# MIT-SPARK/Hydra-GNN

Hardware: AMD Instinct MI355X
Metric: scene-graphs/sec (fwd+bwd) MP3D hetero batch (higher is better)
Workload: dtype f32

## Files before the change

hydra-gnn_amd/csrc/front.hip:

```cpp
#include "device_fns.h"
#ifdef HMP_KTIME
#define PS_KT(i)                                                                           \
  do {                                                                                     \
    if (threadIdx.x == 0 && part == 0 && dir == 0 && J.ei == front_kt_ei) front_kt_slot(i); \
  } while (0)
namespace hmp {
__device__ const void* front_kt_ei;
__device__ void front_kt_slot(int i);
}
#endif
#include "plan_small.h"

namespace hmp {

KT_DEFINE(front)
#ifdef HMP_KTIME
__device__ void front_kt_slot(int i) { kt_buf[i] = wall_clock64(); }
#endif

typedef float f32x16 __attribute__((ext_vector_type(16)));

constexpr int FT = 64;
constexpr int FBK = 128;
constexpr int FLD = FBK + 2;
constexpr int FSTAGES = 3;
constexpr int F_STAGE_FLOATS = 2 * 2 * FT * FLD;
constexpr int F_RED_FLOATS = 16 * 16 * 64;
constexpr int F_GEMM_FLOATS = F_STAGE_FLOATS > F_RED_FLOATS ? F_STAGE_FLOATS : F_RED_FLOATS;
constexpr int F_SEG_OFF = F_GEMM_FLOATS * 4;
constexpr int F_GEMM_BYTES = F_SEG_OFF + FR_MAX_SEG * (int)sizeof(FrontSeg);
constexpr int F_LDS_BYTES = PS_LDS_BYTES > F_GEMM_BYTES ? PS_LDS_BYTES : F_GEMM_BYTES;

template <int VEC>
__device__ __forceinline__ float4 fr_ld4(const float* p, bool second_ok) {
  if (VEC == 4) return *reinterpret_cast<const float4*>(p);
  const float2 a = *reinterpret_cast<const float2*>(p);
  const float2 b = *reinterpret_cast<const float2*>(p + (second_ok ? 2 : 0));
  return make_float4(a.x, a.y, b.x, b.y);
}

template <int VEC, int NSRC>
__device__ __forceinline__ void front_gemm_tile(const FrontProb& P, const FrontSeg* __restrict__ sseg, const float* __restrict__ params,
                                                int tm, int tn, float* lds) {
  const int tid = threadIdx.x, lane = tid & 63, w = __builtin_amdgcn_readfirstlane(tid >> 6);
  const int m0 = tm * FT, n0 = tn * FT;
  const int k4 = (tid & 31) * 4;
  const float* arow[2];
  const float* brow[2][NSRC];
  int bn[2];
#pragma unroll
  for (int i = 0; i < 2; ++i) {
    const int row = (tid >> 5) + 32 * i;
    arow[i] = P.A + (int64_t)min(m0 + row, P.M - 1) * P.lda;
    const int c = n0 + row;
    int si = 0;
    while (si + 1 < P.n_seg && c >= sseg[si + 1].col0) ++si;
    const FrontSeg& S = sseg[si];
    const int br = c - S.col0;
    const bool blive = c < P.N && br >= 0 && br < S.rows;
    bn[i] = blive ? S.nsrc : 0;
#pragma unroll
    for (int q = 0; q < NSRC; ++q) brow[i][q] = params + S.off[q < S.nsrc ? q : 0] + (int64_t)(blive ? br : 0) * S.ld;
  }
  const int n_stage = (P.K + FBK - 1) / FBK;
  float4 ra[FSTAGES][2], rb[FSTAGES][2];
#pragma unroll
  for (int s = 0; s < FSTAGES; ++s) {
    const int gk = s * FBK + k4;
    const bool klive = s < n_stage && gk < P.K;
    const int kc = klive ? gk : 0;
    const bool sec = kc + 2 < P.K;
    const bool m1 = klive && gk + 1 < P.K, m2 = klive && gk + 2 < P.K, m3 = klive && gk + 3 < P.K;
#pragma unroll
    for (int i = 0; i < 2; ++i) {
      const float4 a = fr_ld4<VEC>(arow[i] + kc, sec);
      float4 b = fr_ld4<VEC>(brow[i][0] + kc, sec);
#pragma unroll
      for (int q = 1; q < NSRC; ++q) {
        const float4 t = fr_ld4<VEC>(brow[i][q] + kc, sec);
        if (q < bn[i]) { b.x += t.x; b.y += t.y; b.z += t.z; b.w += t.w; }
      }
      const bool bl = bn[i] > 0;
      ra[s][i] = make_float4(klive ? a.x : 0.f, m1 ? a.y : 0.f, m2 ? a.z : 0.f, m3 ? a.w : 0.f);
      rb[s][i] = make_float4(klive && bl ? b.x : 0.f, m1 && bl ? b.y : 0.f, m2 && bl ? b.z : 0.f, m3 && bl ? b.w : 0.f);
    }
  }
  KT(2);
  KTW(3);
  const int kg = w >> 2, sub = w & 3, wm = sub & 1, wn = sub >> 1;
  f32x16 acc;
#pragma unroll
  for (int i = 0; i < 16; ++i) acc[i] = 0.f;
  auto put = [&](int s) {
    float* As = lds + (s & 1) * (2 * FT * FLD);
    float* Bs = As + FT * FLD;
#pragma unroll
    for (int i = 0; i < 2; ++i) {
      const int row = (tid >> 5) + 32 * i;
      float2* pa = reinterpret_cast<float2*>(As + row * FLD + k4);
      float2* pb = reinterpret_cast<float2*>(Bs + row * FLD + k4);
      pa[0] = make_float2(ra[s][i].x, ra[s][i].y); pa[1] = make_float2(ra[s][i].z, ra[s][i].w);
      pb[0] = make_float2(rb[s][i].x, rb[s][i].y); pb[1] = make_float2(rb[s][i].z, rb[s][i].w);
    }
  };
  put(0);
  KT(5);
  __syncthreads();
  KT(6);
#pragma unroll
  for (int s = 0; s < FSTAGES; ++s) {
    if (s >= n_stage) break;
    if (s + 1 < FSTAGES && s + 1 < n_stage) put(s + 1);
    const float* As = lds + (s & 1) * (2 * FT * FLD);
    const float* Bs = As + FT * FLD;
    const int klen = min(FBK, P.K - s * FBK);
    const int nk = min(max(klen - kg * 32, 0), 32);
    const float* ap = As + (wm * 32 + (lane & 31)) * FLD + kg * 32 + (lane >> 5);
    const float* bp = Bs + (wn * 32 + (lane & 31)) * FLD + kg * 32 + (lane >> 5);
    if (nk == 32) {
#pragma unroll
      for (int h = 0; h < 2; ++h) {
        float av[8], bv[8];
#pragma unroll
        for (int i = 0; i < 8; ++i) {
          av[i] = ap[16 * h + 2 * i];
          bv[i] = bp[16 * h + 2 * i];
        }
#pragma unroll
        for (int i = 0; i < 8; ++i) acc = __builtin_amdgcn_mfma_f32_32x32x2f32(av[i], bv[i], acc, 0, 0, 0);
      }
    } else {
      for (int kk = 0; kk < nk; kk += 2) acc = __builtin_amdgcn_mfma_f32_32x32x2f32(ap[kk], bp[kk], acc, 0, 0, 0);
    }
    if (s == 0) KT(7);
    if (s == 1) KT(14);
    __syncthreads();
    if (s == 0) KT(13);
    if (s == 1) KT(15);
  }
  KT(4);
  float* red = lds;
#pragma unroll
  for (int i = 0; i < 16; ++i) red[(w * 16 + i) * 64 + lane] = acc[i];
  __syncthreads();
  const int col = n0 + wn * 32 + (lane & 31);
#pragma unroll
  for (int j = 0; j < 4; ++j) {
    const int i = 4 * kg + j;
    const float v = (red[((0 * 4 + sub) * 16 + i) * 64 + lane] + red[((1 * 4 + sub) * 16 + i) * 64 + lane]) +
                    (red[((2 * 4 + sub) * 16 + i) * 64 + lane] + red[((3 * 4 + sub) * 16 + i) * 64 + lane]);
    const int row = m0 + wm * 32 + j + 8 * kg + 4 * (lane >> 5);
    if (row < P.M && col < P.N) P.C[(int64_t)row * P.ldc + col] = v;
  }
}

template <int VEC>
__device__ __forceinline__ void front_gemm_v(const FrontProb& P, const FrontSeg* sseg, const float* params, int tm, int tn, float* lds) {
  switch (P.max_nsrc) {
    case 1: front_gemm_tile<VEC, 1>(P, sseg, params, tm, tn, lds); break;
    case 2: front_gemm_tile<VEC, 2>(P, sseg, params, tm, tn, lds); break;
    case 3: front_gemm_tile<VEC, 3>(P, sseg, params, tm, tn, lds); break;
    default: front_gemm_tile<VEC, FR_MAX_SRC>(P, sseg, params, tm, tn, lds); break;
  }
}

__global__ __launch_bounds__(1024) void front_kernel(const FrontArgs a) {
  __shared__ __attribute__((aligned(16))) char lds[F_LDS_BYTES];
  const int blk = blockIdx.x;
  if (blk < a.gemm_blocks) {
    KT(0);
    int pi = 0;
    while (pi + 1 < a.n_prob && blk >= a.prob_start[pi + 1]) ++pi;
    karg_warm<(sizeof(FrontProb) + 63) / 64 + 1>((int)offsetof(FrontArgs, prob) + pi * (int)sizeof(FrontProb), (int)sizeof(FrontProb));
    const FrontProb& P = a.prob[pi];
    const int local = blk - P.blk_start;
    const int tm = local / P.tiles_n, tn = local % P.tiles_n;
    FrontSeg* sseg = reinterpret_cast<FrontSeg*>(lds + F_SEG_OFF);
    if ((int)threadIdx.x < P.n_seg) sseg[threadIdx.x] = P.seg[threadIdx.x];
    __syncthreads();
    if (P.vec == 4) front_gemm_v<4>(P, sseg, a.params, tm, tn, reinterpret_cast<float*>(lds));
    else front_gemm_v<2>(P, sseg, a.params, tm, tn, reinterpret_cast<float*>(lds));
    KT(1);
    return;
  }
  if (blk < a.gemm_blocks + a.plan_blocks) {
    const int pb = blk - a.gemm_blocks;
    int jd = 0;
    while (jd + 1 < 2 * a.n_jobs && pb >= a.part_start[jd + 1]) ++jd;
    const FrontJob& F = a.job[jd >> 1];
    int* wsi = reinterpret_cast<int*>(a.ws);
    PlanJob J;
    J.ei = F.ei; J.E = F.E; J.n_src = F.n_src; J.n_dst = F.n_dst;
    J.rowptr = wsi + F.rowptr; J.col = wsi + F.col; J.eid = wsi + F.eid;
    J.t_rowptr = wsi + F.t_rowptr; J.t_col = wsi + F.t_col; J.t_pos = nullptr;
    J.degf = reinterpret_cast<float*>(wsi + F.degf);
    J.gp_dst = F.gp_dst; J.gp_src = F.gp_src; J.gp_edge = F.gp_edge; J.n_graphs = F.n_graphs;
    J.cnt_in = J.cnt_out = J.cur_in = J.cur_out = nullptr;
    J.tmpc_in = J.tmpc_out = nullptr;
    J.tmp_in = wsi + F.tmp_in; J.tmp_out = wsi + F.tmp_out; J.t_eid = wsi + F.t_eid; J.pos_of_eid = wsi + F.pos_of_eid;
#ifdef HMP_KTIME
    if (threadIdx.x == 0 && pb == 0) front_kt_ei = a.job[0].ei;
#endif
    const bool last = pb + 1 == a.part_start[jd + 1];
    if (a.plan_rc) plan_small_part<true>(J, jd & 1, pb - a.part_start[jd], a.rows_per_part[jd], last, a.need_tpos, a.status, lds);
    else plan_small_part<false>(J, jd & 1, pb - a.part_start[jd], a.rows_per_part[jd], last, a.need_tpos, a.status, lds);
    return;
  }
  const int kb = blk - a.gemm_blocks - a.plan_blocks;
  if (a.step_ctr && kb == 0 && threadIdx.x == 0) {
    const int t = *a.step_ctr + 1;
    *a.step_ctr = t;
    if (a.step_mirror) *a.step_mirror = t;
  }
  const int2 m = a.pack_map[kb];
  pack_item(a.segs[m.x], m.y + (int)(threadIdx.x >> 6), a.params, a.packed);
}

int front_launch(FrontArgs& a, hipStream_t st) {
  int start = 0;
  for (int i = 0; i < a.n_prob; ++i) {
    FrontProb& P = a.prob[i];
    HMP_CHECK_ARG(P.K >= 4 && P.K <= FSTAGES * FBK && (P.K & 1) == 0 && P.M > 0 && P.N > 0, "front: projection K %d unsupported", P.K);
    HMP_CHECK_ARG(P.n_seg >= 1 && P.n_seg <= FR_MAX_SEG, "front: %d segments", P.n_seg);
    const uintptr_t pa = reinterpret_cast<uintptr_t>(P.A), pp = reinterpret_cast<uintptr_t>(a.params);
    HMP_CHECK_ARG((pa & 7) == 0 && (P.lda & 1) == 0 && (pp & 15) == 0, "front: operands must be 8-byte aligned with even leading dimensions");
    int vec = ((pa & 15) == 0 && (P.lda & 3) == 0) ? 4 : 2;
    P.max_nsrc = 1;
    for (int s = 0; s < P.n_seg; ++s) {
      const FrontSeg& S = P.seg[s];
      HMP_CHECK_ARG(S.nsrc >= 1 && S.nsrc <= FR_MAX_SRC && (S.ld & 1) == 0, "front: segment with %d sources / ld %d", S.nsrc, S.ld);
      P.max_nsrc = S.nsrc > P.max_nsrc ? S.nsrc : P.max_nsrc;
      if (S.ld & 3) vec = 2;
      for (int q = 0; q < S.nsrc; ++q) {
        HMP_CHECK_ARG((S.off[q] & 1) == 0, "front: parameter offset not 8-byte aligned");
        if (S.off[q] & 3) vec = 2;
      }
    }
    P.vec = vec;
    P.tiles_m = cdiv(P.M, FT);
    P.tiles_n = cdiv(P.N, FT);
    P.blk_start = start;
    a.prob_start[i] = start;
    start += P.tiles_m * P.tiles_n;
  }
  a.gemm_blocks = start;
  const int total = a.gemm_blocks + a.plan_blocks + a.pack_blocks;
  if (total == 0) return HMP_OK;
  hipLaunchKernelGGL(front_kernel, dim3(total), dim3(1024), 0, st, a);
  HMP_LAUNCH_CHECK();
  return HMP_OK;
}

}
```

hydra-gnn_amd/csrc/plan_small.h:

```cpp
#pragma once
#include "kernels.h"

namespace hmp {

constexpr int PS_ROWS = 1024;
constexpr int PS_TMP = 12 * 1024;
constexpr int PS_UB = 8;
constexpr int64_t PS_MAX_EDGES = 65536;

struct PlanSmallArgs {
  PlanBatch pb;
  int part_start[2 * HMP_MAX_EDGE_TYPES + 1];
  int rows_per_part[2 * HMP_MAX_EDGE_TYPES];
};

constexpr int PS_ROWS_SLICED = 256;
#ifndef PS_KT
#define PS_KT(i)
#endif
constexpr int PS_RC = 24;

constexpr int PS_LDS_BYTES = (PS_ROWS + PS_ROWS + 1 + 2 * PS_TMP + 16 + 2 + 1 + 4) * 4 + PS_TMP * 2;

template <bool RC>
__device__ __forceinline__ void plan_small_part(const PlanJob& J, int dir, int part, int rpp, bool last_part, int need_tpos, int* status,
                                                char* lds) {
  int* cnt = reinterpret_cast<int*>(lds);
  int* lrow = cnt + PS_ROWS;
  int* ltmp = lrow + PS_ROWS + 1;
  int* lcol = ltmp + PS_TMP;
  int* wsum = lcol + PS_TMP;
  int* s_scal = wsum + 16;
  unsigned short* lkey = reinterpret_cast<unsigned short*>(s_scal + 7);
  int& s_base = s_scal[0];
  int& s_total = s_scal[1];
  const int tid = threadIdx.x, lane = tid & 63, w = tid >> 6;
  const int n_rows = dir ? J.n_src : J.n_dst;
  const int r0 = part * rpp;
  const int r1 = min(n_rows, r0 + rpp);
  const int nr = max(r1 - r0, 0);
  const int E = (int)J.E;
  const int64_t* __restrict__ es = J.ei;
  const int64_t* __restrict__ ed = J.ei + J.E;
  const int n_src = J.n_src, n_dst = J.n_dst;

  PS_KT(8);
  for (int i = tid; i < PS_ROWS; i += 1024) cnt[i] = 0;
  const bool sliced = J.gp_edge != nullptr && nr > 0;
  int bad = 0;
  if (tid == 0) { s_scal[3] = 0; s_scal[4] = sliced ? 0 : E; s_scal[5] = 0; s_scal[6] = n_rows; }
  __syncthreads();
  if (sliced) {
    const int64_t* __restrict__ gp = dir ? J.gp_src : J.gp_dst;
    for (int g = tid; g < J.n_graphs; g += 1024) {
      const int64_t a = gp[g], b = gp[g + 1];
      const int64_t ea = J.gp_edge[g], eb = J.gp_edge[g + 1];
      if (a <= r0 && r0 < b) { s_scal[3] = (int)ea; s_scal[5] = (int)a; }
      if (a < r1 && r1 <= b) { s_scal[4] = (int)eb; s_scal[6] = (int)b; }
      if (g + 1 == J.n_graphs && (b != n_rows || eb != E)) bad = 2;
    }
    __syncthreads();
  }
  const int e_lo = __builtin_amdgcn_readfirstlane(min(max(s_scal[3], 0), E));
  const int e_hi = __builtin_amdgcn_readfirstlane(min(max(s_scal[4], e_lo), E));
  const int key_lo = __builtin_amdgcn_readfirstlane(s_scal[5]), key_hi = __builtin_amdgcn_readfirstlane(s_scal[6]);
  int below = tid == 0 ? e_lo : 0;
  int cs[RC ? PS_RC : 1], cd[RC ? PS_RC : 1];
  if constexpr (RC) {
#pragma unroll
    for (int i = 0; i < PS_RC; ++i) {
      const int e = e_lo + tid + i * 1024;
      const int ec = max(min(e, e_hi - 1), 0);
      int64_t s = -1, d = -1;
      if (e_hi > e_lo) { s = es[ec]; d = ed[ec]; }
      const bool in = e < e_hi;
      const bool ok = in && s >= 0 && s < n_src && d >= 0 && d < n_dst;
      if (in && !ok) bad |= 1;
      cs[i] = ok ? (int)s : -1;
      cd[i] = (int)d;
    }
#pragma unroll
    for (int i = 0; i < PS_RC; ++i) {
      if (cs[i] < 0) continue;
      const int key = dir ? cs[i] : cd[i];
      if (key < key_lo || key >= key_hi) bad |= 2;
      if (key < r0) ++below;
      else if (key < r1) atomicAdd(&cnt[key - r0], 1);
    }
  } else
  for (int e0 = e_lo + tid; e0 < e_hi; e0 += PS_UB * 1024) {
    int64_t sv[PS_UB], dv[PS_UB];
#pragma unroll
    for (int u = 0; u < PS_UB; ++u) {
      const int e = min(e0 + u * 1024, e_hi - 1);
      sv[u] = es[e];
      dv[u] = ed[e];
    }
#pragma unroll
    for (int u = 0; u < PS_UB; ++u) {
      if (e0 + u * 1024 >= e_hi) break;
      const int64_t s = sv[u], d = dv[u];
      if (s < 0 || s >= n_src || d < 0 || d >= n_dst) { bad |= 1; continue; }
      const int key = (int)(dir ? s : d);
      if (key < key_lo || key >= key_hi) bad |= 2;
      if (key < r0) ++below;
      else if (key < r1) atomicAdd(&cnt[key - r0], 1);
    }
  }
  PS_KT(9);
  if ((bad & 1) && status && (sliced || (part == 0 && dir == 0))) atomicOr(status, 1);
  if ((bad & 2) && status) atomicOr(status, 4);
#pragma unroll
  for (int o = 32; o > 0; o >>= 1) below += __shfl_xor(below, o);
  if (lane == 0) wsum[w] = below;
  __syncthreads();
  if (tid == 0) {
    int b = 0;
    for (int q = 0; q < 16; ++q) b += wsum[q];
    s_base = b;
  }
  __syncthreads();
  const int base = s_base;
  {
    const int v = tid < nr ? cnt[tid] : 0;
    int x = v;
#pragma unroll
    for (int o = 1; o < 64; o <<= 1) {
      const int y = __shfl_up(x, o);
      if (lane >= o) x += y;
    }
    __syncthreads();
    if (lane == 63) wsum[w] = x;
    __syncthreads();
    int woff = 0;
    for (int q = 0; q < w; ++q) woff += wsum[q];
    const int excl = woff + x - v;
    if (tid < nr) {
      lrow[tid] = excl;
      (dir ? J.t_rowptr : J.rowptr)[r0 + tid] = base + excl;
      if (!dir && J.degf) J.degf[r0 + tid] = 1.f / (float)(v > 1 ? v : 1);
      cnt[tid] = 0;
    }
    if (tid == 1023) s_total = woff + x;
    __syncthreads();
    if (tid == 0) {
      lrow[nr] = s_total;
      if (last_part) (dir ? J.t_rowptr : J.rowptr)[n_rows] = base + s_total;
    }
  }
  __syncthreads();
  PS_KT(10);
  const int total = s_total;
  const bool in_lds = total <= PS_TMP;
  int* __restrict__ gtmp = (dir ? J.tmp_out : J.tmp_in) + base;
  if constexpr (RC) {
#pragma unroll
    for (int i = 0; i < PS_RC; ++i) {
      if (cs[i] < 0) continue;
      const int key = dir ? cs[i] : cd[i];
      if (key < r0 || key >= r1) continue;
      const int e = e_lo + tid + i * 1024;
      const int slot = lrow[key - r0] + atomicAdd(&cnt[key - r0], 1);
      if (in_lds) {
        ltmp[slot] = e;
        lcol[slot] = dir ? cd[i] : cs[i];
        lkey[slot] = (unsigned short)(key - r0);
      } else {
        gtmp[slot] = e;
      }
    }
  } else
  for (int e0 = e_lo + tid; e0 < e_hi; e0 += PS_UB * 1024) {
    int64_t sv[PS_UB], dv[PS_UB];
#pragma unroll
    for (int u = 0; u < PS_UB; ++u) {
      const int e = min(e0 + u * 1024, e_hi - 1);
      sv[u] = es[e];
      dv[u] = ed[e];
    }
#pragma unroll
    for (int u = 0; u < PS_UB; ++u) {
      const int e = e0 + u * 1024;
      if (e >= e_hi) break;
      const int64_t s = sv[u], d = dv[u];
      if (s < 0 || s >= n_src || d < 0 || d >= n_dst) continue;
      const int key = (int)(dir ? s : d);
      if (key < r0 || key >= r1) continue;
      const int slot = lrow[key - r0] + atomicAdd(&cnt[key - r0], 1);
      if (in_lds) {
        ltmp[slot] = e;
        lcol[slot] = (int)(dir ? d : s);
        lkey[slot] = (unsigned short)(key - r0);
      } else {
        gtmp[slot] = e;
      }
    }
  }
  __syncthreads();
  PS_KT(11);
  if (in_lds) {
    for (int q = tid; q < total; q += 1024) {
      const int r = lkey[q];
      const int b = lrow[r], en = lrow[r + 1];
      const int mine = ltmp[q];
      int rank = 0;
      for (int i = b; i < en; ++i) rank += (ltmp[i] < mine) ? 1 : 0;
      const int pos = base + b + rank;
      if (dir == 0) {
        J.eid[pos] = mine;
        J.col[pos] = lcol[q];
        if (need_tpos) J.pos_of_eid[mine] = pos;
      } else {
        if (need_tpos) J.t_eid[pos] = mine;
        J.t_col[pos] = lcol[q];
      }
    }
  } else {
    for (int q = tid; q < total; q += 1024) {
      int lo = 0, hi = nr - 1;
      while (lo < hi) {
        const int mid = (lo + hi + 1) >> 1;
        if (lrow[mid] <= q) lo = mid; else hi = mid - 1;
      }
      const int b = lrow[lo], en = lrow[lo + 1];
      const int mine = gtmp[q];
      int rank = 0;
      for (int i = b; i < en; ++i) rank += (gtmp[i] < mine) ? 1 : 0;
      const int pos = base + b + rank;
      if (dir == 0) {
        J.eid[pos] = mine;
        J.col[pos] = (int)es[mine];
        if (need_tpos) J.pos_of_eid[mine] = pos;
      } else {
        if (need_tpos) J.t_eid[pos] = mine;
        J.t_col[pos] = (int)ed[mine];
      }
    }
  }
  PS_KT(12);
}


template <bool RC>
__device__ __forceinline__ void plan_small_block(const PlanSmallArgs& a, int* status, int blk, char* lds) {
  int jd = 0;
  while (jd + 1 < 2 * a.pb.n && blk >= a.part_start[jd + 1]) ++jd;
  plan_small_part<RC>(a.pb.j[jd >> 1], jd & 1, blk - a.part_start[jd], a.rows_per_part[jd], blk + 1 == a.part_start[jd + 1],
                      a.pb.need_tpos, status, lds);
}

inline int plan_small_layout(const PlanBatch& pb, int* part_start , int* rows_per_part ) {
  int blocks = 0;
  for (int jd = 0; jd < 2 * pb.n; ++jd) {
    const PlanJob& J = pb.j[jd >> 1];
    const int nrows = (jd & 1) ? J.n_src : J.n_dst;
    const int rows_max = J.gp_edge ? PS_ROWS_SLICED : PS_ROWS;
    const int parts = nrows > 0 ? cdiv(nrows, rows_max) : 1;
    part_start[jd] = blocks;
    rows_per_part[jd] = nrows > 0 ? cdiv(nrows, parts) : 1;
    blocks += parts;
  }
  part_start[2 * pb.n] = blocks;
  return blocks;
}
inline bool plan_small_fits_rc(const PlanBatch& pb) {
  int64_t emax = 0;
  bool sliced = pb.n > 0;
  for (int j = 0; j < pb.n; ++j) {
    emax = pb.j[j].E > emax ? pb.j[j].E : emax;
    sliced = sliced && (pb.j[j].gp_edge != nullptr || pb.j[j].E == 0);
  }
  if (sliced) return false;
  return emax <= (int64_t)PS_RC * 1024;
}

}
```

Measured before the change: 373,300.

## Drop LDS segment staging and barriers; keep edges in registers in plan

The front GEMM now resolves each column's parameter segment straight from kernel arguments with a branchless unrolled select. This removes the LDS copy of the segment table and a block barrier, and it uses 32-bit offsets for the B rows. In the small planning kernel, the base and total prefix computations are merged into one scan pass using separate wsum/wscan buffers, which cuts several __syncthreads. When the edge range fits in one unrolled pass, the source and destination indices are kept in registers so the second edge read from global memory is skipped. The costs are higher register pressure, and the 32-bit offsets could overflow if the parameter buffers are very large.

```diff
diff --git a/hydra-gnn_amd/csrc/front.hip b/hydra-gnn_amd/csrc/front.hip
--- a/hydra-gnn_amd/csrc/front.hip
+++ b/hydra-gnn_amd/csrc/front.hip
@@ -27,8 +27,7 @@
 constexpr int F_STAGE_FLOATS = 2 * 2 * FT * FLD;
 constexpr int F_RED_FLOATS = 16 * 16 * 64;
 constexpr int F_GEMM_FLOATS = F_STAGE_FLOATS > F_RED_FLOATS ? F_STAGE_FLOATS : F_RED_FLOATS;
-constexpr int F_SEG_OFF = F_GEMM_FLOATS * 4;
-constexpr int F_GEMM_BYTES = F_SEG_OFF + FR_MAX_SEG * (int)sizeof(FrontSeg);
+constexpr int F_GEMM_BYTES = F_GEMM_FLOATS * 4;
 constexpr int F_LDS_BYTES = PS_LDS_BYTES > F_GEMM_BYTES ? PS_LDS_BYTES : F_GEMM_BYTES;
 
 template <int VEC>
@@ -40,27 +39,36 @@
 }
 
 template <int VEC, int NSRC>
-__device__ __forceinline__ void front_gemm_tile(const FrontProb& P, const FrontSeg* __restrict__ sseg, const float* __restrict__ params,
-                                                int tm, int tn, float* lds) {
+__device__ __forceinline__ void front_gemm_tile(const FrontProb& P, const float* __restrict__ params, int tm, int tn, float* lds) {
   const int tid = threadIdx.x, lane = tid & 63, w = __builtin_amdgcn_readfirstlane(tid >> 6);
   const int m0 = tm * FT, n0 = tn * FT;
   const int k4 = (tid & 31) * 4;
   const float* arow[2];
-  const float* brow[2][NSRC];
+  uint32_t brow[2][NSRC];
   int bn[2];
 #pragma unroll
   for (int i = 0; i < 2; ++i) {
     const int row = (tid >> 5) + 32 * i;
     arow[i] = P.A + (int64_t)min(m0 + row, P.M - 1) * P.lda;
     const int c = n0 + row;
-    int si = 0;
-    while (si + 1 < P.n_seg && c >= sseg[si + 1].col0) ++si;
-    const FrontSeg& S = sseg[si];
-    const int br = c - S.col0;
-    const bool blive = c < P.N && br >= 0 && br < S.rows;
-    bn[i] = blive ? S.nsrc : 0;
-#pragma unroll
-    for (int q = 0; q < NSRC; ++q) brow[i][q] = params + S.off[q < S.nsrc ? q : 0] + (int64_t)(blive ? br : 0) * S.ld;
+    int col0 = P.seg[0].col0, rows = P.seg[0].rows, nsrc = P.seg[0].nsrc, ld = P.seg[0].ld;
+    uint32_t off[NSRC];
+#pragma unroll
+    for (int q = 0; q < NSRC; ++q) off[q] = q < P.seg[0].nsrc ? P.seg[0].off[q] : P.seg[0].off[0];
+    bool go = true;
+#pragma unroll
+    for (int si = 1; si < FR_MAX_SEG; ++si) {
+      const FrontSeg& G = P.seg[si];
+      go = go && si < P.n_seg && c >= G.col0;
+      col0 = go ? G.col0 : col0; rows = go ? G.rows : rows; nsrc = go ? G.nsrc : nsrc; ld = go ? G.ld : ld;
+#pragma unroll
+      for (int q = 0; q < NSRC; ++q) off[q] = go ? (q < G.nsrc ? G.off[q] : G.off[0]) : off[q];
+    }
+    const int br = c - col0;
+    const bool blive = c < P.N && br >= 0 && br < rows;
+    bn[i] = blive ? nsrc : 0;
+#pragma unroll
+    for (int q = 0; q < NSRC; ++q) brow[i][q] = off[q] + (uint32_t)((blive ? br : 0) * ld);
   }
   const int n_stage = (P.K + FBK - 1) / FBK;
   float4 ra[FSTAGES][2], rb[FSTAGES][2];
@@ -74,10 +82,10 @@
 #pragma unroll
     for (int i = 0; i < 2; ++i) {
       const float4 a = fr_ld4<VEC>(arow[i] + kc, sec);
-      float4 b = fr_ld4<VEC>(brow[i][0] + kc, sec);
+      float4 b = fr_ld4<VEC>(params + (brow[i][0] + kc), sec);
 #pragma unroll
       for (int q = 1; q < NSRC; ++q) {
-        const float4 t = fr_ld4<VEC>(brow[i][q] + kc, sec);
+        const float4 t = fr_ld4<VEC>(params + (brow[i][q] + kc), sec);
         if (q < bn[i]) { b.x += t.x; b.y += t.y; b.z += t.z; b.w += t.w; }
       }
       const bool bl = bn[i] > 0;
@@ -155,12 +163,12 @@
 }
 
 template <int VEC>
-__device__ __forceinline__ void front_gemm_v(const FrontProb& P, const FrontSeg* sseg, const float* params, int tm, int tn, float* lds) {
+__device__ __forceinline__ void front_gemm_v(const FrontProb& P, const float* params, int tm, int tn, float* lds) {
   switch (P.max_nsrc) {
-    case 1: front_gemm_tile<VEC, 1>(P, sseg, params, tm, tn, lds); break;
-    case 2: front_gemm_tile<VEC, 2>(P, sseg, params, tm, tn, lds); break;
-    case 3: front_gemm_tile<VEC, 3>(P, sseg, params, tm, tn, lds); break;
-    default: front_gemm_tile<VEC, FR_MAX_SRC>(P, sseg, params, tm, tn, lds); break;
+    case 1: front_gemm_tile<VEC, 1>(P, params, tm, tn, lds); break;
+    case 2: front_gemm_tile<VEC, 2>(P, params, tm, tn, lds); break;
+    case 3: front_gemm_tile<VEC, 3>(P, params, tm, tn, lds); break;
+    default: front_gemm_tile<VEC, FR_MAX_SRC>(P, params, tm, tn, lds); break;
   }
 }
 
@@ -171,15 +179,13 @@
     KT(0);
     int pi = 0;
     while (pi + 1 < a.n_prob && blk >= a.prob_start[pi + 1]) ++pi;
+    pi = __builtin_amdgcn_readfirstlane(pi);
     karg_warm<(sizeof(FrontProb) + 63) / 64 + 1>((int)offsetof(FrontArgs, prob) + pi * (int)sizeof(FrontProb), (int)sizeof(FrontProb));
-    const FrontProb& P = a.prob[pi];
+    const FrontProb& P = ((const FrontArgs*)__builtin_amdgcn_kernarg_segment_ptr())->prob[pi];
     const int local = blk - P.blk_start;
     const int tm = local / P.tiles_n, tn = local % P.tiles_n;
-    FrontSeg* sseg = reinterpret_cast<FrontSeg*>(lds + F_SEG_OFF);
-    if ((int)threadIdx.x < P.n_seg) sseg[threadIdx.x] = P.seg[threadIdx.x];
-    __syncthreads();
-    if (P.vec == 4) front_gemm_v<4>(P, sseg, a.params, tm, tn, reinterpret_cast<float*>(lds));
-    else front_gemm_v<2>(P, sseg, a.params, tm, tn, reinterpret_cast<float*>(lds));
+    if (P.vec == 4) front_gemm_v<4>(P, a.params, tm, tn, reinterpret_cast<float*>(lds));
+    else front_gemm_v<2>(P, a.params, tm, tn, reinterpret_cast<float*>(lds));
     KT(1);
     return;
   }
diff --git a/hydra-gnn_amd/csrc/plan_small.h b/hydra-gnn_amd/csrc/plan_small.h
--- a/hydra-gnn_amd/csrc/plan_small.h
+++ b/hydra-gnn_amd/csrc/plan_small.h
@@ -20,7 +20,7 @@
 #endif
 constexpr int PS_RC = 24;
 
-constexpr int PS_LDS_BYTES = (PS_ROWS + PS_ROWS + 1 + 2 * PS_TMP + 16 + 2 + 1 + 4) * 4 + PS_TMP * 2;
+constexpr int PS_LDS_BYTES = (PS_ROWS + PS_ROWS + 1 + 2 * PS_TMP + 16 + 16 + 2 + 1 + 4) * 4 + PS_TMP * 2;
 
 template <bool RC>
 __device__ __forceinline__ void plan_small_part(const PlanJob& J, int dir, int part, int rpp, bool last_part, int need_tpos, int* status,
@@ -30,10 +30,9 @@
   int* ltmp = lrow + PS_ROWS + 1;
   int* lcol = ltmp + PS_TMP;
   int* wsum = lcol + PS_TMP;
-  int* s_scal = wsum + 16;
+  int* wscan = wsum + 16;
+  int* s_scal = wscan + 16;
   unsigned short* lkey = reinterpret_cast<unsigned short*>(s_scal + 7);
-  int& s_base = s_scal[0];
-  int& s_total = s_scal[1];
   const int tid = threadIdx.x, lane = tid & 63, w = tid >> 6;
   const int n_rows = dir ? J.n_src : J.n_dst;
   const int r0 = part * rpp;
@@ -66,6 +65,12 @@
   const int key_lo = __builtin_amdgcn_readfirstlane(s_scal[5]), key_hi = __builtin_amdgcn_readfirstlane(s_scal[6]);
   int below = tid == 0 ? e_lo : 0;
   int cs[RC ? PS_RC : 1], cd[RC ? PS_RC : 1];
+  const bool keep = !RC && e_hi - e_lo <= PS_UB * 1024;
+  int ks[RC ? 1 : PS_UB], kd[RC ? 1 : PS_UB];
+  if constexpr (!RC) {
+#pragma unroll
+    for (int u = 0; u < PS_UB; ++u) { ks[u] = -1; kd[u] = -1; }
+  }
   if constexpr (RC) {
 #pragma unroll
     for (int i = 0; i < PS_RC; ++i) {
@@ -101,6 +106,7 @@
       if (e0 + u * 1024 >= e_hi) break;
       const int64_t s = sv[u], d = dv[u];
       if (s < 0 || s >= n_src || d < 0 || d >= n_dst) { bad |= 1; continue; }
+      ks[u] = (int)s; kd[u] = (int)d;
       const int key = (int)(dir ? s : d);
       if (key < key_lo || key >= key_hi) bad |= 2;
       if (key < r0) ++below;
@@ -114,13 +120,7 @@
   for (int o = 32; o > 0; o >>= 1) below += __shfl_xor(below, o);
   if (lane == 0) wsum[w] = below;
   __syncthreads();
-  if (tid == 0) {
-    int b = 0;
-    for (int q = 0; q < 16; ++q) b += wsum[q];
-    s_base = b;
-  }
-  __syncthreads();
-  const int base = s_base;
+  int base = 0, total = 0;
   {
     const int v = tid < nr ? cnt[tid] : 0;
     int x = v;
@@ -129,11 +129,16 @@
       const int y = __shfl_up(x, o);
       if (lane >= o) x += y;
     }
-    __syncthreads();
-    if (lane == 63) wsum[w] = x;
+    if (lane == 63) wscan[w] = x;
     __syncthreads();
     int woff = 0;
-    for (int q = 0; q < w; ++q) woff += wsum[q];
+#pragma unroll
+    for (int q = 0; q < 16; ++q) {
+      base += wsum[q];
+      woff += q < w ? wscan[q] : 0;
+      total += wscan[q];
+    }
+    base = __builtin_amdgcn_readfirstlane(base); total = __builtin_amdgcn_readfirstlane(total); woff = __builtin_amdgcn_readfirstlane(woff);
     const int excl = woff + x - v;
     if (tid < nr) {
       lrow[tid] = excl;
@@ -141,16 +146,13 @@
       if (!dir && J.degf) J.degf[r0 + tid] = 1.f / (float)(v > 1 ? v : 1);
       cnt[tid] = 0;
     }
-    if (tid == 1023) s_total = woff + x;
-    __syncthreads();
     if (tid == 0) {
-      lrow[nr] = s_total;
-      if (last_part) (dir ? J.t_rowptr : J.rowptr)[n_rows] = base + s_total;
+      lrow[nr] = total;
+      if (last_part) (dir ? J.t_rowptr : J.rowptr)[n_rows] = base + total;
     }
   }
   __syncthreads();
   PS_KT(10);
-  const int total = s_total;
   const bool in_lds = total <= PS_TMP;
   int* __restrict__ gtmp = (dir ? J.tmp_out : J.tmp_in) + base;
   if constexpr (RC) {
@@ -167,6 +169,21 @@
         lkey[slot] = (unsigned short)(key - r0);
       } else {
         gtmp[slot] = e;
+      }
+    }
+  } else if (keep) {
+#pragma unroll
+    for (int u = 0; u < PS_UB; ++u) {
+      if (ks[u] < 0) continue;
+      const int key = dir ? ks[u] : kd[u];
+      if (key < r0 || key >= r1) continue;
+      const int slot = lrow[key - r0] + atomicAdd(&cnt[key - r0], 1);
+      if (in_lds) {
+        ltmp[slot] = e_lo + tid + u * 1024;
+        lcol[slot] = dir ? kd[u] : ks[u];
+        lkey[slot] = (unsigned short)(key - r0);
+      } else {
+        gtmp[slot] = e_lo + tid + u * 1024;
       }
     }
   } else
```

New measurement: 369,500. 0.99x the previous value.
